# olehskip/resnet.c

Measured on AMD Instinct MI355X. Metric: images/sec ResNet-50 224x224 fp32 batch=256, higher is better.
Workload: dtype f32; 1 GPU; resnet50 fp32 forward, batch 256 per GPU, 224x224 (BASELINE.json configs[2]); global_batch=256, batch_per_gpu=256, mode=fused conv+bn+relu(+add) epilogues, streams_per_gpu=2, streams_configured=library default, front_parts=1, parallelism=batch split over 1 GPU(s), weights replicated, no collective

## Files before the change

resnet.c_amd/csrc/rn_chain.hip:

```cpp
#include "rn_conv_params.h"
#include "rn_lds_dma.h"

using namespace rn_gemm;
using namespace rn_dma;

namespace {

struct ChainParams {
    const void *t2;
    const void *x;
    void *y;
    const void *w3;
    const float *sc3, *sh3;
    void *t1;
    const void *w1;
    const float *sc1, *sh1;
    int M, nsteps;
    int t2_bytes, x_bytes, y_bytes, t1_bytes;
};

typedef bf16_t bf16x4 __attribute__((ext_vector_type(4)));

template <int MID>
struct Geo {
    static constexpr int C = 4 * MID;
    static constexpr int WAVES = MID == 64 ? 8 : 4;
    static constexpr int ROWS = MID == 64 ? 64 : 32;
    static constexpr int PF = ROWS / 32;
    static constexpr int CF1 = C / (32 * WAVES);
    static constexpr int KT2 = MID / 64;
    static constexpr int T2B = ROWS * MID * 2;
    static constexpr int XB = ROWS * C * 2;
    static constexpr int oT2 = 0, oX = 2 * T2B, oY = oX + 2 * XB, oS = oY + XB;
    static constexpr int LDS = oS + (2 * C + 512) * 4;
};

template <int MID, int N1, bool DUAL>
__global__ __launch_bounds__(64 * Geo<MID>::WAVES) void chain_kernel(const ChainParams p)
{
    using G = Geo<MID>;
    constexpr int C = G::C, ROWS = G::ROWS, PF = G::PF, CF1 = G::CF1, THREADS = 64 * G::WAVES;
    constexpr int N1F = N1 / 32;
    static_assert(!DUAL || MID == 64, "pair chain: 64 mid channels");
    static_assert(PF * N1F <= G::WAVES, "one fragment of the second product per wave");
    __shared__ __attribute__((aligned(16))) char lds[G::LDS];
    float *const ssl = reinterpret_cast<float *>(lds + G::oS);
    const int t = threadIdx.x, lane = t & 63;
    const int wave = __builtin_amdgcn_readfirstlane(t >> 6);
    const int li = lane & 31, lh = lane >> 5;

    int nst, s0;
    dealt_range((unsigned)p.nsteps, gridDim.x, blockIdx.x, &nst, &s0);

    const int pf2 = wave % PF, cf2 = wave / PF;
    const bool has2 = cf2 < N1F;
    constexpr int K3S = (DUAL ? 2 : 1) * MID / 16;
    constexpr int K1S = C / 16;
    i32x4 w3r[CF1][K3S], w1r[K1S];
#pragma unroll
    for (int f = 0; f < CF1; ++f) {
        const char *r3 = static_cast<const char *>(p.w3) + (size_t)(32 * (CF1 * wave + f) + li) * (K3S * 32) + lh * 16;
#pragma unroll
        for (int ks = 0; ks < K3S; ++ks) w3r[f][ks] = *reinterpret_cast<const i32x4 *>(r3 + ks * 32);
    }
    {
        const char *r1 = static_cast<const char *>(p.w1) + (size_t)(32 * (has2 ? cf2 : 0) + li) * (K1S * 32) + lh * 16;
#pragma unroll
        for (int s = 0; s < K1S; ++s) w1r[s] = *reinterpret_cast<const i32x4 *>(r1 + s * 32);
    }
    for (int i = t; i < C; i += THREADS) {
        ssl[i] = p.sc3 ? p.sc3[i] : 1.f;
        ssl[C + i] = p.sh3 ? p.sh3[i] : -0.f;
    }
    for (int i = t; i < N1; i += THREADS) {
        ssl[2 * C + i] = p.sc1 ? p.sc1[i] : 1.f;
        ssl[2 * C + 256 + i] = p.sh1 ? p.sh1[i] : -0.f;
    }

    const i32x4 srd_t2 = make_srd(p.t2, p.t2_bytes);
    const i32x4 srd_x = make_srd(p.x, p.x_bytes);
    const __amdgpu_buffer_rsrc_t rsrc_y = make_rsrc(p.y, p.y_bytes);
    const __amdgpu_buffer_rsrc_t rsrc_t1 = make_rsrc(p.t1, p.t1_bytes);
    const unsigned lds_base = (unsigned)(uintptr_t)((lds_void *)lds);

    auto fetch = [&](int s, int buf) {
        const int m0 = (s0 + s) * ROWS;
        const bool live = s < nst;
        constexpr int T2P = G::KT2 * ROWS / 8;
#pragma unroll
        for (int j = 0; j < T2P / G::WAVES; ++j) {
            const int q = G::WAVES * j + wave, kt = q / (ROWS / 8), r = 8 * (q % (ROWS / 8)) + (lane >> 3);
            const int pc = lane & 7, m = m0 + r;
            dma16((live && m < p.M) ? m * (MID * 2) + kt * 128 + (RN_SWZ(pc, r) << 4) : kOob, srd_t2, 0,
                  lds_base + (unsigned)(G::oT2 + buf * G::T2B + q * 1024));
        }
        if constexpr (DUAL) {
#pragma unroll
            for (int j = 0; j < T2P / G::WAVES; ++j) {
                const int q = G::WAVES * j + wave, r = 8 * q + (lane >> 3), pc = lane & 7, m = m0 + r;
                dma16((live && m < p.M) ? m * 128 + (RN_SWZ(pc, r) << 4) : kOob, srd_x, 0,
                      lds_base + (unsigned)(G::oX + buf * G::XB + q * 1024));
            }
        } else {
            constexpr int XP = G::XB / 1024, SPR = C / 8;
#pragma unroll
            for (int j = 0; j < XP / G::WAVES; ++j) {
                const int q = G::WAVES * j + wave, g = 64 * q + lane;
                const int r = g / SPR, sl = g % SPR, m = m0 + r;
                const int c = (sl & ~15) | ((sl & 15) ^ (r & 15));
                dma16((live && m < p.M) ? m * (C * 2) + (c << 4) : kOob, srd_x, 0,
                      lds_base + (unsigned)(G::oX + buf * G::XB + q * 1024));
            }
        }
    };

    fetch(0, 0);
    for (int s = 0; s < nst; ++s) {
        const int buf = s & 1;
        const int m0 = (s0 + s) * ROWS;
        wait_and_barrier<0>();
        if constexpr (MID == 64) fetch(s + 1, buf ^ 1);

        f32x16 acc[PF][CF1];
#pragma unroll
        for (int pf = 0; pf < PF; ++pf)
#pragma unroll
            for (int f = 0; f < CF1; ++f)
#pragma unroll
                for (int e = 0; e < 16; ++e) acc[pf][f][e] = 0.f;
#pragma unroll
        for (int ks = 0; ks < K3S; ++ks) {
#pragma unroll
            for (int pf = 0; pf < PF; ++pf) {
                const int r = 32 * pf + li;
                const bool second = DUAL && ks >= MID / 16;
                const int kk = second ? ks - MID / 16 : ks;
                const char *src = second ? lds + G::oX + buf * G::XB : lds + G::oT2 + buf * G::T2B;
                const i32x4 px = *reinterpret_cast<const i32x4 *>(
                    src + (kk >> 2) * (ROWS * 128) + r * 128 + (RN_SWZ(2 * (kk & 3) + lh, r) << 4));
#pragma unroll
                for (int f = 0; f < CF1; ++f)
                    acc[pf][f] = __builtin_amdgcn_mfma_f32_32x32x16_bf16(__builtin_bit_cast(bf16x8, w3r[f][ks]),
                                                                         __builtin_bit_cast(bf16x8, px), acc[pf][f], 0, 0, 0);
            }
        }
        if constexpr (MID != 64) fetch(s + 1, buf ^ 1);
#pragma unroll
        for (int pf = 0; pf < PF; ++pf)
#pragma unroll
            for (int f = 0; f < CF1; ++f) {
                const int r = 32 * pf + li, cf = CF1 * wave + f;
                unsigned d[4][2];
#pragma unroll
                for (int j = 0; j < 4; ++j) {
                    const int c4 = 32 * cf + 8 * j + 4 * lh;
                    const float4 sc = *reinterpret_cast<const float4 *>(ssl + c4);
                    const float4 sh = *reinterpret_cast<const float4 *>(ssl + C + c4);
                    float4 v = affine4(acc[pf][f], j, sc, sh);
                    if constexpr (!DUAL) {
                        const int chunk = 4 * cf + j;
                        const bf16x4 rv = *reinterpret_cast<const bf16x4 *>(
                            lds + G::oX + buf * G::XB + r * (C * 2) +
                            (((chunk & ~15) | ((chunk & 15) ^ (r & 15))) << 4) + 8 * lh);
                        v.x = v.x + (float)rv[0], v.y = v.y + (float)rv[1], v.z = v.z + (float)rv[2], v.w = v.w + (float)rv[3];
                    }
                    pack_bf16x4(relu4(v), d[j]);
                }
#pragma unroll
                for (int h = 0; h < 2; ++h) {
                    const auto x0 = __builtin_amdgcn_permlane32_swap(d[2 * h][0], d[2 * h + 1][0], false, false);
                    const auto x1 = __builtin_amdgcn_permlane32_swap(d[2 * h][1], d[2 * h + 1][1], false, false);
                    const int cy = 4 * cf + 2 * h + lh;
                    *reinterpret_cast<i32x4 *>(lds + G::oY + (cy >> 3) * (ROWS * 128) + r * 128 +
                                               (RN_SWZ(cy & 7, r) << 4)) =
                        i32x4{(int)x0[0], (int)x1[0], (int)x0[1], (int)x1[1]};
                }
            }
        __syncthreads();

#pragma unroll
        for (int i = 0; i < ROWS * (C / 8) / THREADS; ++i) {
            const int g = t + i * THREADS, r = g / (C / 8), c = g % (C / 8), m = m0 + r;
            const i32x4 v = *reinterpret_cast<const i32x4 *>(lds + G::oY + (c >> 3) * (ROWS * 128) + r * 128 +
                                                             (RN_SWZ(c & 7, r) << 4));
            __builtin_amdgcn_raw_buffer_store_b128(__builtin_bit_cast(u32x4, v), rsrc_y,
                                                   m < p.M ? m * (C * 2) + (c << 4) : kOob, 0, 0);
        }

        if (has2) {
            const int r = 32 * pf2 + li;
            f32x16 a2;
#pragma unroll
            for (int e = 0; e < 16; ++e) a2[e] = 0.f;
#pragma unroll
            for (int s2 = 0; s2 < K1S; ++s2) {
                const i32x4 px = *reinterpret_cast<const i32x4 *>(
                    lds + G::oY + (s2 >> 2) * (ROWS * 128) + r * 128 + (RN_SWZ(2 * (s2 & 3) + lh, r) << 4));
                a2 = __builtin_amdgcn_mfma_f32_32x32x16_bf16(__builtin_bit_cast(bf16x8, w1r[s2]),
                                                             __builtin_bit_cast(bf16x8, px), a2, 0, 0, 0);
            }
            unsigned d[4][2];
#pragma unroll
            for (int j = 0; j < 4; ++j) {
                const int c4 = 32 * cf2 + 8 * j + 4 * lh;
                const float4 sc = *reinterpret_cast<const float4 *>(ssl + 2 * C + c4);
                const float4 sh = *reinterpret_cast<const float4 *>(ssl + 2 * C + 256 + c4);
                pack_bf16x4(affine4_relu(a2, j, sc, sh), d[j]);
            }
            const int m = m0 + r;
#pragma unroll
            for (int h = 0; h < 2; ++h) {
                const auto x0 = __builtin_amdgcn_permlane32_swap(d[2 * h][0], d[2 * h + 1][0], false, false);
                const auto x1 = __builtin_amdgcn_permlane32_swap(d[2 * h][1], d[2 * h + 1][1], false, false);
                const u32x4 o = {x0[0], x1[0], x0[1], x1[1]};
                __builtin_amdgcn_raw_buffer_store_b128(
                    o, rsrc_t1, m < p.M ? (m * N1 + 32 * cf2 + 16 * h + 8 * lh) * 2 : kOob, 0, 0);
            }
        }
    }
}

template <int MID, int N1, bool DUAL>
void chain_go(rn_ctx *ctx, const ChainParams &p)
{
    const int blocks = p.nsteps < 256 ? p.nsteps : 256;
    chain_kernel<MID, N1, DUAL><<<dim3(blocks), dim3(64 * Geo<MID>::WAVES), 0, ctx->stream>>>(p);
}

constexpr int k32XY = 0, k32XYB = 64 * 1024, k32T2 = 2 * k32XYB, k32T2B = 64 * 256;
constexpr int k32S = k32T2 + k32T2B, k32Lds = k32S + (512 + 256) * 4;

template <int N1>
__global__ __launch_bounds__(512) void chain32_kernel(const ChainParams p)
{
    constexpr int ROWS = 64, N1F = N1 / 32;
    __shared__ __attribute__((aligned(16))) char lds[k32Lds];
    float *const ssl = reinterpret_cast<float *>(lds + k32S);
    const int t = threadIdx.x, lane = t & 63;
    const int wave = __builtin_amdgcn_readfirstlane(t >> 6);
    const int li = lane & 31, lh = lane >> 5;
    int nst, s0;
    dealt_range((unsigned)p.nsteps, gridDim.x, blockIdx.x, &nst, &s0);
    const int pf2 = wave & 1, cf2 = wave >> 1;
    const bool has2 = cf2 < N1F;
    u32x4 w3r[2][4], w1r[8][4];
    {
        const char *r3 = static_cast<const char *>(p.w3) + (size_t)(32 * wave + li) * 256 + lh * 16;
#pragma unroll
        for (int kt = 0; kt < 2; ++kt)
#pragma unroll
            for (int ks = 0; ks < 4; ++ks) w3r[kt][ks] = *reinterpret_cast<const u32x4 *>(r3 + kt * 128 + ks * 32);
        const char *r1 = static_cast<const char *>(p.w1) + (size_t)(32 * (has2 ? cf2 : 0) + li) * 1024 + lh * 16;
#pragma unroll
        for (int kt = 0; kt < 8; ++kt)
#pragma unroll
            for (int ks = 0; ks < 4; ++ks) w1r[kt][ks] = *reinterpret_cast<const u32x4 *>(r1 + kt * 128 + ks * 32);
    }
    for (int i = t; i < 256; i += 512) {
        ssl[i] = p.sc3 ? p.sc3[i] : 1.f;
        ssl[256 + i] = p.sh3 ? p.sh3[i] : -0.f;
    }
    for (int i = t; i < N1; i += 512) {
        ssl[512 + i] = p.sc1 ? p.sc1[i] : 1.f;
        ssl[640 + i] = p.sh1 ? p.sh1[i] : -0.f;
    }
    const i32x4 srd_t2 = make_srd(p.t2, p.t2_bytes);
    const i32x4 srd_x = make_srd(p.x, p.x_bytes);
    const __amdgpu_buffer_rsrc_t rsrc_y = make_rsrc(p.y, p.y_bytes);
    const __amdgpu_buffer_rsrc_t rsrc_t1 = make_rsrc(p.t1, p.t1_bytes);
    const unsigned lds_base = (unsigned)(uintptr_t)((lds_void *)lds);
    const int prow = lane >> 3, pc = lane & 7;

    auto fetch_t2 = [&](int s) {
        const int m0 = (s0 + s) * ROWS;
#pragma unroll
        for (int j = 0; j < 2; ++j) {
            const int q = 8 * j + wave, r = 8 * (q & 7) + prow, m = m0 + r;
            dma16((s < nst && m < p.M) ? m * 256 + (q >> 3) * 128 + (RN_SWZ(pc, r) << 4) : kOob, srd_t2, 0,
                  lds_base + (unsigned)(k32T2 + q * 1024));
        }
    };
    auto fetch_x = [&](int s, int buf) {
        const int m0 = (s0 + s) * ROWS;
#pragma unroll
        for (int j = 0; j < 8; ++j) {
            const int q = 8 * j + wave, r = 8 * (q & 7) + prow, m = m0 + r;
            dma16((s < nst && m < p.M) ? m * 1024 + (q >> 3) * 128 + (RN_SWZ(pc, r) << 4) : kOob, srd_x, 0,
                  lds_base + (unsigned)(k32XY + buf * k32XYB + q * 1024));
        }
    };

    fetch_t2(0);
    fetch_x(0, 0);
    for (int s = 0; s < nst; ++s) {
        const int buf = s & 1;
        const int m0 = (s0 + s) * ROWS;
        char *const xy = lds + k32XY + buf * k32XYB;
        wait_and_barrier<0>();
        fetch_x(s + 1, buf ^ 1);

        f32x16 acc[2];
#pragma unroll
        for (int pf = 0; pf < 2; ++pf)
#pragma unroll
            for (int e = 0; e < 16; ++e) acc[pf][e] = 0.f;
#pragma unroll
        for (int pf = 0; pf < 2; ++pf)
#pragma unroll
            for (int kt = 0; kt < 2; ++kt)
#pragma unroll
                for (int ks = 0; ks < 4; ++ks) {
                    const int r = 32 * pf + li;
                    const u32x4 px = *reinterpret_cast<const u32x4 *>(
                        lds + k32T2 + kt * 8192 + r * 128 + (RN_SWZ(2 * ks + lh, r) << 4));
#pragma unroll
                    for (int j = 0; j < 4; ++j)
                        acc[pf] = __builtin_amdgcn_mfma_f32_32x32x2f32(__uint_as_float(w3r[kt][ks][j]),
                                                                        __uint_as_float(px[j]), acc[pf], 0, 0, 0);
                }
#pragma unroll
        for (int pf = 0; pf < 2; ++pf) {
            const int r = 32 * pf + li;
#pragma unroll
            for (int g = 0; g < 4; ++g) {
                const int c4 = 32 * wave + 8 * g + 4 * lh;
                const float4 sc = *reinterpret_cast<const float4 *>(ssl + c4);
                const float4 sh = *reinterpret_cast<const float4 *>(ssl + 256 + c4);
                float4 *slot = reinterpret_cast<float4 *>(xy + wave * 8192 + r * 128 + (RN_SWZ(2 * g + lh, r) << 4));
                const float4 rv = *slot;
                *slot = affine4_add_relu(acc[pf], g, sc, sh, rv);
            }
        }
        __syncthreads();
        fetch_t2(s + 1);

        {
            constexpr bool kSplit = N1F == 2;
            const int tt = kSplit ? t - 256 : t;
            if (!kSplit || wave >= 4) {
#pragma unroll 1
                for (int i0 = 0; i0 < (kSplit ? 16 : 8); i0 += 4) {
#pragma unroll
                    for (int i = i0; i < i0 + 4; ++i) {
                        const int g = tt + i * (kSplit ? 256 : 512), r = g >> 6, c = g & 63, m = m0 + r;
                        const u32x4 v = *reinterpret_cast<const u32x4 *>(xy + (c >> 3) * 8192 + r * 128 +
                                                                         (RN_SWZ(c & 7, r) << 4));
                        __builtin_amdgcn_raw_buffer_store_b128(v, rsrc_y, m < p.M ? m * 1024 + (c << 4) : kOob, 0, 0);
                    }
                }
            }
        }

        if (has2) {
            const int r = 32 * pf2 + li;
            f32x16 a2;
#pragma unroll
            for (int e = 0; e < 16; ++e) a2[e] = 0.f;
#pragma unroll
            for (int kt = 0; kt < 8; ++kt)
#pragma unroll
                for (int ks = 0; ks < 4; ++ks) {
                    const u32x4 px = *reinterpret_cast<const u32x4 *>(
                        xy + kt * 8192 + r * 128 + (RN_SWZ(2 * ks + lh, r) << 4));
#pragma unroll
                    for (int j = 0; j < 4; ++j)
                        a2 = __builtin_amdgcn_mfma_f32_32x32x2f32(__uint_as_float(w1r[kt][ks][j]), __uint_as_float(px[j]),
                                                                  a2, 0, 0, 0);
                }
            const int m = m0 + r;
#pragma unroll
            for (int g = 0; g < 4; ++g) {
                const int c4 = 32 * cf2 + 8 * g + 4 * lh;
                const float4 sc = *reinterpret_cast<const float4 *>(ssl + 512 + c4);
                const float4 sh = *reinterpret_cast<const float4 *>(ssl + 640 + c4);
                const u32x4 o = __builtin_bit_cast(u32x4, affine4_relu(a2, g, sc, sh));
                __builtin_amdgcn_raw_buffer_store_b128(o, rsrc_t1, m < p.M ? (m * N1 + c4) * 4 : kOob, 0, 0);
            }
        }
    }
}

constexpr int kP32Y = 0, kP32W1 = 64 * 1024, kP32T2 = 128 * 1024, kP32X2 = 144 * 1024, kP32Lds = 160 * 1024;

__global__ __launch_bounds__(512) void chain32_pair_kernel(const ChainParams p)
{
    constexpr int ROWS = 64;
    __shared__ __attribute__((aligned(16))) char lds[kP32Lds];
    const int t = threadIdx.x, lane = t & 63;
    const int wave = __builtin_amdgcn_readfirstlane(t >> 6);
    const int li = lane & 31, lh = lane >> 5;
    int nst, s0;
    dealt_range((unsigned)p.nsteps, gridDim.x, blockIdx.x, &nst, &s0);
    const int pf2 = wave & 1, cf2 = wave >> 1;
    const bool has2 = cf2 < 2;
    u32x4 w3r[4][4];
    {
        const char *r3 = static_cast<const char *>(p.w3) + (size_t)(32 * wave + li) * 512 + lh * 16;
#pragma unroll
        for (int kt = 0; kt < 4; ++kt)
#pragma unroll
            for (int ks = 0; ks < 4; ++ks) w3r[kt][ks] = *reinterpret_cast<const u32x4 *>(r3 + kt * 128 + ks * 32);
    }
    const i32x4 srd_t2 = make_srd(p.t2, p.t2_bytes);
    const i32x4 srd_x = make_srd(p.x, p.x_bytes);
    const i32x4 srd_w1 = make_srd(p.w1, 64 * 256 * 4);
    const __amdgpu_buffer_rsrc_t rsrc_y = make_rsrc(p.y, p.y_bytes);
    const __amdgpu_buffer_rsrc_t rsrc_t1 = make_rsrc(p.t1, p.t1_bytes);
    const unsigned lds_base = (unsigned)(uintptr_t)((lds_void *)lds);
    const int prow = lane >> 3, pc = lane & 7;

#pragma unroll
    for (int j = 0; j < 8; ++j) {
        const int q = 8 * j + wave, r = 8 * (q & 7) + prow;
        dma16(r * 1024 + (q >> 3) * 128 + (RN_SWZ(pc, r) << 4), srd_w1, 0,
              lds_base + (unsigned)(kP32W1 + q * 1024));
    }
    auto fetch_in = [&](int s) {
        const int m0 = (s0 + s) * ROWS;
#pragma unroll
        for (int j = 0; j < 2; ++j) {
            const int q = 8 * j + wave, r = 8 * (q & 7) + prow, m = m0 + r;
            const int off = (s < nst && m < p.M) ? m * 256 + (q >> 3) * 128 + (RN_SWZ(pc, r) << 4) : kOob;
            dma16(off, srd_t2, 0, lds_base + (unsigned)(kP32T2 + q * 1024));
            dma16(off, srd_x, 0, lds_base + (unsigned)(kP32X2 + q * 1024));
        }
    };

    fetch_in(0);
    for (int s = 0; s < nst; ++s) {
        const int m0 = (s0 + s) * ROWS;
        wait_and_barrier<0>();

        f32x16 acc[2];
#pragma unroll
        for (int pf = 0; pf < 2; ++pf)
#pragma unroll
            for (int e = 0; e < 16; ++e) acc[pf][e] = 0.f;
#pragma unroll
        for (int pf = 0; pf < 2; ++pf)
#pragma unroll
            for (int kt = 0; kt < 4; ++kt)
#pragma unroll
                for (int ks = 0; ks < 4; ++ks) {
                    const int r = 32 * pf + li;
                    const u32x4 px = *reinterpret_cast<const u32x4 *>(
                        lds + (kt < 2 ? kP32T2 : kP32X2) + (kt & 1) * 8192 + r * 128 + (RN_SWZ(2 * ks + lh, r) << 4));
#pragma unroll
                    for (int j = 0; j < 4; ++j)
                        acc[pf] = __builtin_amdgcn_mfma_f32_32x32x2f32(__uint_as_float(w3r[kt][ks][j]),
                                                                        __uint_as_float(px[j]), acc[pf], 0, 0, 0);
                }
#pragma unroll
        for (int pf = 0; pf < 2; ++pf) {
            const int r = 32 * pf + li;
#pragma unroll
            for (int g = 0; g < 4; ++g) {
                const int c4 = 32 * wave + 8 * g + 4 * lh;
                const float4 sh = p.sh3 ? *reinterpret_cast<const float4 *>(p.sh3 + c4) : make_float4(-0.f, -0.f, -0.f, -0.f);
                const float4 o = affine4_relu(acc[pf], g, make_float4(1.f, 1.f, 1.f, 1.f), sh);
                *reinterpret_cast<float4 *>(lds + kP32Y + wave * 8192 + r * 128 + (RN_SWZ(2 * g + lh, r) << 4)) = o;
            }
        }
        __syncthreads();
        fetch_in(s + 1);

        if (wave >= 4) {
#pragma unroll 1
            for (int i0 = 0; i0 < 16; i0 += 4) {
#pragma unroll
                for (int i = i0; i < i0 + 4; ++i) {
                    const int g = t - 256 + i * 256, r = g >> 6, c = g & 63, m = m0 + r;
                    const u32x4 v = *reinterpret_cast<const u32x4 *>(lds + kP32Y + (c >> 3) * 8192 + r * 128 +
                                                                     (RN_SWZ(c & 7, r) << 4));
                    __builtin_amdgcn_raw_buffer_store_b128(v, rsrc_y, m < p.M ? m * 1024 + (c << 4) : kOob, 0, 0);
                }
            }
        }

        if (has2) {
            const int r = 32 * pf2 + li, wr = 32 * cf2 + li;
            f32x16 a2;
#pragma unroll
            for (int e = 0; e < 16; ++e) a2[e] = 0.f;
#pragma unroll
            for (int kt = 0; kt < 8; ++kt)
#pragma unroll
                for (int ks = 0; ks < 4; ++ks) {
                    const u32x4 px = *reinterpret_cast<const u32x4 *>(
                        lds + kP32Y + kt * 8192 + r * 128 + (RN_SWZ(2 * ks + lh, r) << 4));
                    const u32x4 wv = *reinterpret_cast<const u32x4 *>(
                        lds + kP32W1 + kt * 8192 + wr * 128 + (RN_SWZ(2 * ks + lh, wr) << 4));
#pragma unroll
                    for (int j = 0; j < 4; ++j)
                        a2 = __builtin_amdgcn_mfma_f32_32x32x2f32(__uint_as_float(wv[j]), __uint_as_float(px[j]), a2, 0, 0, 0);
                }
            const int m = m0 + r;
#pragma unroll
            for (int g = 0; g < 4; ++g) {
                const int c4 = 32 * cf2 + 8 * g + 4 * lh;
                const float4 sc = p.sc1 ? *reinterpret_cast<const float4 *>(p.sc1 + c4) : make_float4(1.f, 1.f, 1.f, 1.f);
                const float4 sh = p.sh1 ? *reinterpret_cast<const float4 *>(p.sh1 + c4) : make_float4(-0.f, -0.f, -0.f, -0.f);
                const u32x4 o = __builtin_bit_cast(u32x4, affine4_relu(a2, g, sc, sh));
                __builtin_amdgcn_raw_buffer_store_b128(o, rsrc_t1, m < p.M ? (m * 64 + c4) * 4 : kOob, 0, 0);
            }
        }
    }
}

int chain_launch(rn_ctx *ctx, const char *what, int dtype, const void *t2, const void *x, bool dual, void *y,
                 const void *w3, const float *scale3, const float *shift3, void *t1, const void *w1,
                 const float *scale1, const float *shift1, uint64_t rows, uint64_t mid_channels,
                 uint64_t channels, uint64_t next_mid)
{
    if (rows == 0) return RN_OK;
    RN_REQUIRE(ctx, dtype == RN_DTYPE_BF16 || dtype == RN_DTYPE_F32, "unknown dtype");
    RN_REQUIRE(ctx, t2 && x && y && w3 && t1 && w1, "null tensor");
    RN_REQUIRE(ctx, ((reinterpret_cast<uintptr_t>(t2) | reinterpret_cast<uintptr_t>(x) | reinterpret_cast<uintptr_t>(y) |
                      reinterpret_cast<uintptr_t>(t1) | reinterpret_cast<uintptr_t>(w3) | reinterpret_cast<uintptr_t>(w1) |
                      reinterpret_cast<uintptr_t>(scale3) | reinterpret_cast<uintptr_t>(shift3) |
                      reinterpret_cast<uintptr_t>(scale1) | reinterpret_cast<uintptr_t>(shift1)) & 15) == 0,
               "tensors, panels and scale / shift vectors must be 16-byte aligned");
    RN_REQUIRE(ctx, y != t1 && y != t2 && y != x && t1 != t2 && t1 != x, "y and t1 must not alias each other or an input");
    const bool s1 = mid_channels == 64 && channels == 256 && (next_mid == 64 || next_mid == 128);
    const bool s2 = mid_channels == 128 && channels == 512 && next_mid == 128 && !dual && dtype == RN_DTYPE_BF16;
    RN_REQUIRE(ctx, s1 || s2, "shapes: 64 -> 256 -> 64 | 128 channels, or (bf16) 128 -> 512 -> 128");
    RN_REQUIRE(ctx, !(dual && dtype == RN_DTYPE_F32 && next_mid != 64), "fp32 pair chain: next_mid 64");
    const uint64_t es = rn_elem_size(dtype);
    RN_REQUIRE(ctx, rows * channels * es < (1ull << 31), "tensor too large");
    if (dtype == RN_DTYPE_F32) {
        ChainParams q;
        q.t2 = t2, q.x = x, q.y = y, q.w3 = w3, q.sc3 = scale3, q.sh3 = shift3;
        q.t1 = t1, q.w1 = w1, q.sc1 = scale1, q.sh1 = shift1;
        q.M = (int)rows;
        q.nsteps = (int)((rows + 63) / 64);
        q.t2_bytes = (int)(rows * 256), q.x_bytes = q.y_bytes = (int)(rows * 1024), q.t1_bytes = (int)(rows * next_mid * 4);
        const dim3 grid(q.nsteps < 256 ? q.nsteps : 256), block(512);
        if (dual) {
            q.x_bytes = (int)(rows * 256);
            chain32_pair_kernel<<<grid, block, 0, ctx->stream>>>(q);
        } else if (next_mid == 64)
            chain32_kernel<64><<<grid, block, 0, ctx->stream>>>(q);
        else
            chain32_kernel<128><<<grid, block, 0, ctx->stream>>>(q);
        return rn_after_launch(ctx, what);
    }
    ChainParams p;
    p.t2 = t2, p.x = x, p.y = y, p.w3 = w3, p.sc3 = scale3, p.sh3 = shift3;
    p.t1 = t1, p.w1 = w1, p.sc1 = scale1, p.sh1 = shift1;
    p.M = (int)rows;
    const uint64_t step = s1 ? 64 : 32;
    p.nsteps = (int)((rows + step - 1) / step);
    p.t2_bytes = (int)(rows * mid_channels * 2), p.x_bytes = (int)(rows * (dual ? 128 : channels * 2));
    p.y_bytes = (int)(rows * channels * 2), p.t1_bytes = (int)(rows * next_mid * 2);
    if (s2)
        chain_go<128, 128, false>(ctx, p);
    else if (dual)
        next_mid == 64 ? chain_go<64, 64, true>(ctx, p) : chain_go<64, 128, true>(ctx, p);
    else
        next_mid == 64 ? chain_go<64, 64, false>(ctx, p) : chain_go<64, 128, false>(ctx, p);
    return rn_after_launch(ctx, what);
}

}

extern "C" {

int rn_conv_chain_forward_dt(rn_ctx *ctx, int dtype, const void *t2, const void *residual, void *y,
                             const void *packed_w3, const float *scale3, const float *shift3,
                             void *t1, const void *packed_w1, const float *scale1, const float *shift1,
                             uint64_t rows, uint64_t mid_channels, uint64_t channels, uint64_t next_mid)
{
    RN_ENTER(ctx);
    return chain_launch(ctx, "rn_conv_chain_forward_dt", dtype, t2, residual, false, y, packed_w3, scale3, shift3,
                        t1, packed_w1, scale1, shift1, rows, mid_channels, channels, next_mid);
}

int rn_conv_chain_pair_forward_dt(rn_ctx *ctx, int dtype, const void *t2, const void *x2, void *y,
                                  const void *packed_pair, const float *shift, void *t1,
                                  const void *packed_w1, const float *scale1, const float *shift1,
                                  uint64_t rows, uint64_t mid_channels, uint64_t in2_channels,
                                  uint64_t channels, uint64_t next_mid)
{
    RN_ENTER(ctx);
    RN_REQUIRE(ctx, in2_channels == 64, "second input: 64 channels");
    return chain_launch(ctx, "rn_conv_chain_pair_forward_dt", dtype, t2, x2, true, y, packed_pair, nullptr, shift,
                        t1, packed_w1, scale1, shift1, rows, mid_channels, channels, next_mid);
}

}
```

Measured before the change: 15230 images/s.

## Overlap conv3 epilogue, y export and DMA waits with MFMA in fp32 chain kernels

Reworks the fp32 chain kernels' per-step schedule. Full vmcnt(0) barriers become partial DMA waits, and the next x prefetch now issues after the first MFMA group. The conv3 BN/residual epilogue for the first row half runs interleaved with the second half's MFMAs, and the y export is split across conv1 MFMA iterations with double-buffered LDS loads. It also reorders the DMA row mapping, hoists scale/shift vectors into registers in the pair kernel, and adds an optional timestamp instrumentation path. The aim is to hide LDS, epilogue and store latency behind matrix ops, at the cost of register pressure and fragile hand-counted waitcnt values.

```diff
diff --git a/resnet.c_amd/csrc/rn_chain.hip b/resnet.c_amd/csrc/rn_chain.hip
--- a/resnet.c_amd/csrc/rn_chain.hip
+++ b/resnet.c_amd/csrc/rn_chain.hip
@@ -230,8 +230,104 @@
 constexpr int k32XY = 0, k32XYB = 64 * 1024, k32T2 = 2 * k32XYB, k32T2B = 64 * 256;
 constexpr int k32S = k32T2 + k32T2B, k32Lds = k32S + (512 + 256) * 4;
 
-template <int N1>
-__global__ __launch_bounds__(512) void chain32_kernel(const ChainParams p)
+template <int AFTER>
+__device__ __forceinline__ void wait_dma(bool first)
+{
+    if (first)
+        asm volatile("s_waitcnt vmcnt(0)" ::: "memory");
+    else
+        asm volatile("s_waitcnt vmcnt(%0)" ::"n"(AFTER) : "memory");
+}
+__device__ __forceinline__ void lds_barrier()
+{
+    asm volatile("s_waitcnt lgkmcnt(0)\n\ts_barrier" ::: "memory");
+    __builtin_amdgcn_sched_barrier(0);
+}
+
+__device__ __forceinline__ void settle(float4 &v)
+{
+    asm volatile("" : "+v"(v.x), "+v"(v.y), "+v"(v.z), "+v"(v.w));
+}
+
+template <int NW>
+struct ExportY {
+    const char *lds0;
+    __amdgpu_buffer_rsrc_t rsrc_y;
+    int tile_off, m0, M, first;
+    int lrow, lane_lds, lane_glb;
+    bool whole;
+    __device__ __forceinline__ ExportY(const char *lds0_, int tile_off_, __amdgpu_buffer_rsrc_t rsrc, int m0_, int M_, int first_,
+                                       int lane)
+        : lds0(lds0_), rsrc_y(rsrc), tile_off(tile_off_), m0(m0_), M(M_), first(first_), lrow((lane >> 3) & 1),
+          lane_lds((lane >> 4) * 8192 + lrow * 128 + ((lane & 7) << 4)),
+          lane_glb(lrow * 1024 + (lane >> 4) * 128 + ((lane & 7) << 4)), whole(m0_ + 64 <= M_)
+    {
+    }
+    __device__ __forceinline__ void read(int i0, u32x4 (&v)[4]) const
+    {
+#pragma unroll
+        for (int i = 0; i < 4; ++i) {
+            const int u = first + (i0 + i) * NW, rp = u >> 1;
+            v[i] = *reinterpret_cast<const u32x4 *>(
+                lds0 + (lane_lds ^ (tile_off + (u & 1) * 32768 + rp * 256 + ((rp & 7) << 4))));
+        }
+    }
+    __device__ __forceinline__ void store(int i0, const u32x4 (&v)[4]) const
+    {
+        if (whole) {
+#pragma unroll
+            for (int i = 0; i < 4; ++i) {
+                const int u = first + (i0 + i) * NW, m = m0 + 2 * (u >> 1);
+                __builtin_amdgcn_raw_buffer_store_b128(v[i], rsrc_y, lane_glb, m * 1024 + (u & 1) * 512, 0);
+            }
+        } else {
+#pragma unroll
+            for (int i = 0; i < 4; ++i) {
+                const int u = first + (i0 + i) * NW, m = m0 + 2 * (u >> 1);
+                __builtin_amdgcn_raw_buffer_store_b128(v[i], rsrc_y, m + lrow < M ? m * 1024 + (u & 1) * 512 + lane_glb : kOob, 0, 0);
+            }
+        }
+    }
+    __device__ __forceinline__ void all() const
+    {
+#pragma unroll 1
+        for (int i0 = 0; i0 < 64 / NW; i0 += 4) {
+            u32x4 v[4];
+            read(i0, v);
+            store(i0, v);
+        }
+    }
+};
+
+constexpr int kStampStep = 2, kStampSlots = 9;
+struct Chain32Params : ChainParams {
+    unsigned long long *stamps;
+};
+template <bool STAMP>
+struct Stamps {
+    unsigned long long tk[kStampSlots] = {};
+    __device__ __forceinline__ void at(int s, int slot)
+    {
+        if constexpr (STAMP) {
+            if (s == kStampStep) {
+                __builtin_amdgcn_sched_barrier(0);
+                tk[slot] = __builtin_amdgcn_s_memtime();
+                __builtin_amdgcn_sched_barrier(0);
+            }
+        }
+    }
+    __device__ __forceinline__ void write(unsigned long long *out, int wave, int lane) const
+    {
+        if constexpr (STAMP) {
+            if (out && lane == 0 && tk[kStampSlots - 1])
+#pragma unroll
+                for (int i = 0; i < kStampSlots; ++i) out[((size_t)blockIdx.x * 8 + wave) * 16 + i] = tk[i];
+        }
+    }
+};
+
+template <int N1, bool STAMP>
+__global__ __launch_bounds__(512) void chain32_kernel(const Chain32Params p)
 {
     constexpr int ROWS = 64, N1F = N1 / 32;
     __shared__ __attribute__((aligned(16))) char lds[k32Lds];
@@ -275,8 +371,8 @@
         const int m0 = (s0 + s) * ROWS;
 #pragma unroll
         for (int j = 0; j < 2; ++j) {
-            const int q = 8 * j + wave, r = 8 * (q & 7) + prow, m = m0 + r;
-            dma16((s < nst && m < p.M) ? m * 256 + (q >> 3) * 128 + (RN_SWZ(pc, r) << 4) : kOob, srd_t2, 0,
+            const int q = 8 * j + wave, r = 8 * wave + prow, m = m0 + r;
+            dma16((s < nst && m < p.M) ? m * 256 + (RN_SWZ(pc, r) << 4) : kOob, srd_t2, j * 128,
                   lds_base + (unsigned)(k32T2 + q * 1024));
         }
     };
@@ -284,105 +380,143 @@
         const int m0 = (s0 + s) * ROWS;
 #pragma unroll
         for (int j = 0; j < 8; ++j) {
-            const int q = 8 * j + wave, r = 8 * (q & 7) + prow, m = m0 + r;
-            dma16((s < nst && m < p.M) ? m * 1024 + (q >> 3) * 128 + (RN_SWZ(pc, r) << 4) : kOob, srd_x, 0,
+            const int q = 8 * j + wave, r = 8 * wave + prow, m = m0 + r;
+            dma16((s < nst && m < p.M) ? m * 1024 + (RN_SWZ(pc, r) << 4) : kOob, srd_x, j * 128,
                   lds_base + (unsigned)(k32XY + buf * k32XYB + q * 1024));
         }
     };
 
+    constexpr bool kSplit = N1F == 2;
+    Stamps<STAMP> st;
     fetch_t2(0);
     fetch_x(0, 0);
     for (int s = 0; s < nst; ++s) {
         const int buf = s & 1;
         const int m0 = (s0 + s) * ROWS;
         char *const xy = lds + k32XY + buf * k32XYB;
-        wait_and_barrier<0>();
-        fetch_x(s + 1, buf ^ 1);
+        if (kSplit && wave >= 4)
+            wait_dma<16>(s == 0);
+        else
+            wait_dma<kSplit ? 4 : 12>(s == 0);
+        lds_barrier();
+        st.at(s - 1, 8);
+        st.at(s, 0);
 
         f32x16 acc[2];
 #pragma unroll
         for (int pf = 0; pf < 2; ++pf)
 #pragma unroll
             for (int e = 0; e < 16; ++e) acc[pf][e] = 0.f;
+        st.at(s, 1);
+        auto slot_of = [&](int pf, int g) {
+            const int r = 32 * pf + li;
+            return reinterpret_cast<float4 *>(xy + wave * 8192 + r * 128) + RN_SWZ(2 * g + lh, r);
+        };
+        auto cst = [&](int g, float4 &sc, float4 &sh) {
+            const int c4 = 32 * wave + 8 * g + 4 * lh;
+            sc = *reinterpret_cast<const float4 *>(ssl + c4), sh = *reinterpret_cast<const float4 *>(ssl + 256 + c4);
+        };
+        float4 rv1, sc, sh, rv[4];
 #pragma unroll
         for (int pf = 0; pf < 2; ++pf)
 #pragma unroll
-            for (int kt = 0; kt < 2; ++kt)
-#pragma unroll
-                for (int ks = 0; ks < 4; ++ks) {
-                    const int r = 32 * pf + li;
-                    const u32x4 px = *reinterpret_cast<const u32x4 *>(
-                        lds + k32T2 + kt * 8192 + r * 128 + (RN_SWZ(2 * ks + lh, r) << 4));
-#pragma unroll
-                    for (int j = 0; j < 4; ++j)
-                        acc[pf] = __builtin_amdgcn_mfma_f32_32x32x2f32(__uint_as_float(w3r[kt][ks][j]),
-                                                                        __uint_as_float(px[j]), acc[pf], 0, 0, 0);
-                }
-#pragma unroll
-        for (int pf = 0; pf < 2; ++pf) {
-            const int r = 32 * pf + li;
-#pragma unroll
-            for (int g = 0; g < 4; ++g) {
-                const int c4 = 32 * wave + 8 * g + 4 * lh;
-                const float4 sc = *reinterpret_cast<const float4 *>(ssl + c4);
-                const float4 sh = *reinterpret_cast<const float4 *>(ssl + 256 + c4);
-                float4 *slot = reinterpret_cast<float4 *>(xy + wave * 8192 + r * 128 + (RN_SWZ(2 * g + lh, r) << 4));
-                const float4 rv = *slot;
-                *slot = affine4_add_relu(acc[pf], g, sc, sh, rv);
-            }
-        }
+            for (int gi = 0; gi < 8; ++gi) {
+                const int kt = gi >> 2, ks = gi & 3;
+                const int r = 32 * pf + li;
+                const u32x4 px = *reinterpret_cast<const u32x4 *>(
+                    lds + k32T2 + kt * 8192 + r * 128 + (RN_SWZ(2 * ks + lh, r) << 4));
+                if (pf == 1 && gi <= 4) {
+                    if (gi >= 1) *slot_of(0, gi - 1) = affine4_add_relu(acc[0], gi - 1, sc, sh, rv1);
+                    if (gi <= 3) rv1 = *slot_of(0, gi), cst(gi, sc, sh);
+                    __builtin_amdgcn_sched_barrier(0);
+                }
+                if (pf == 1 && gi == 6) {
+#pragma unroll
+                    for (int g = 0; g < 4; ++g) rv[g] = *slot_of(1, g);
+                    cst(0, sc, sh);
+                    __builtin_amdgcn_sched_barrier(0);
+                }
+#pragma unroll
+                for (int j = 0; j < 4; ++j)
+                    acc[pf] = __builtin_amdgcn_mfma_f32_32x32x2f32(__uint_as_float(w3r[kt][ks][j]),
+                                                                    __uint_as_float(px[j]), acc[pf], 0, 0, 0);
+                if (pf == 1 && (gi <= 4 || gi == 6)) __builtin_amdgcn_sched_barrier(0);
+                if (pf == 0 && gi == 0) {
+                    __builtin_amdgcn_sched_barrier(0);
+                    fetch_x(s + 1, buf ^ 1);
+                    __builtin_amdgcn_sched_barrier(0);
+                }
+            }
+        st.at(s, 2);
+#pragma unroll
+        for (int g = 0; g < 4; ++g) {
+            if (g) cst(g, sc, sh);
+            rv[g] = affine4_add_relu(acc[1], g, sc, sh, rv[g]);
+        }
+#pragma unroll
+        for (int g = 0; g < 4; ++g) *slot_of(1, g) = rv[g];
+        st.at(s, 3);
         __syncthreads();
+        st.at(s, 4);
         fetch_t2(s + 1);
 
-        {
-            constexpr bool kSplit = N1F == 2;
-            const int tt = kSplit ? t - 256 : t;
-            if (!kSplit || wave >= 4) {
-#pragma unroll 1
-                for (int i0 = 0; i0 < (kSplit ? 16 : 8); i0 += 4) {
-#pragma unroll
-                    for (int i = i0; i < i0 + 4; ++i) {
-                        const int g = tt + i * (kSplit ? 256 : 512), r = g >> 6, c = g & 63, m = m0 + r;
-                        const u32x4 v = *reinterpret_cast<const u32x4 *>(xy + (c >> 3) * 8192 + r * 128 +
-                                                                         (RN_SWZ(c & 7, r) << 4));
-                        __builtin_amdgcn_raw_buffer_store_b128(v, rsrc_y, m < p.M ? m * 1024 + (c << 4) : kOob, 0, 0);
-                    }
-                }
-            }
-        }
+        static_assert(kSplit || N1F == 4, "unsplit: every wave has a fragment of conv1 to export beside");
+        if constexpr (kSplit) {
+            if (wave >= 4) ExportY<4>(lds, k32XY + buf * k32XYB, rsrc_y, m0, p.M, wave - 4, lane).all();
+        }
+        const ExportY<8> ex(lds, k32XY + buf * k32XYB, rsrc_y, m0, p.M, wave, lane);
+        u32x4 ev[4];
+        st.at(s, 5);
 
         if (has2) {
             const int r = 32 * pf2 + li;
             f32x16 a2;
 #pragma unroll
             for (int e = 0; e < 16; ++e) a2[e] = 0.f;
-#pragma unroll
-            for (int kt = 0; kt < 8; ++kt)
-#pragma unroll
-                for (int ks = 0; ks < 4; ++ks) {
-                    const u32x4 px = *reinterpret_cast<const u32x4 *>(
-                        xy + kt * 8192 + r * 128 + (RN_SWZ(2 * ks + lh, r) << 4));
-#pragma unroll
-                    for (int j = 0; j < 4; ++j)
-                        a2 = __builtin_amdgcn_mfma_f32_32x32x2f32(__uint_as_float(w1r[kt][ks][j]), __uint_as_float(px[j]),
-                                                                  a2, 0, 0, 0);
-                }
+            const char *const yrow = xy + r * 128;
+            u32x4 px[2];
+            float4 sc1v[4], sh1v[4];
+            px[0] = *reinterpret_cast<const u32x4 *>(yrow + (RN_SWZ(lh, r) << 4));
+#pragma unroll
+            for (int q = 0; q < 32; ++q) {
+                if constexpr (!kSplit) {
+                    if (q == 0 || q == 4) ex.read(q, ev);
+                    if (q == 2 || q == 6) ex.store(q - 2, ev);
+                }
+                if (q == 30) {
+#pragma unroll
+                    for (int g = 0; g < 4; ++g) {
+                        const int c4 = 32 * cf2 + 8 * g + 4 * lh;
+                        sc1v[g] = *reinterpret_cast<const float4 *>(ssl + 512 + c4);
+                        sh1v[g] = *reinterpret_cast<const float4 *>(ssl + 640 + c4);
+                    }
+                }
+                if (q + 1 < 32)
+                    px[(q + 1) & 1] = *reinterpret_cast<const u32x4 *>(
+                        yrow + ((q + 1) >> 2) * 8192 + (RN_SWZ(2 * ((q + 1) & 3) + lh, r) << 4));
+#pragma unroll
+                for (int j = 0; j < 4; ++j)
+                    a2 = __builtin_amdgcn_mfma_f32_32x32x2f32(__uint_as_float(w1r[q >> 2][q & 3][j]),
+                                                              __uint_as_float(px[q & 1][j]), a2, 0, 0, 0);
+            }
+            st.at(s, 6);
             const int m = m0 + r;
 #pragma unroll
             for (int g = 0; g < 4; ++g) {
                 const int c4 = 32 * cf2 + 8 * g + 4 * lh;
-                const float4 sc = *reinterpret_cast<const float4 *>(ssl + 512 + c4);
-                const float4 sh = *reinterpret_cast<const float4 *>(ssl + 640 + c4);
-                const u32x4 o = __builtin_bit_cast(u32x4, affine4_relu(a2, g, sc, sh));
+                const u32x4 o = __builtin_bit_cast(u32x4, affine4_relu(a2, g, sc1v[g], sh1v[g]));
                 __builtin_amdgcn_raw_buffer_store_b128(o, rsrc_t1, m < p.M ? (m * N1 + c4) * 4 : kOob, 0, 0);
             }
         }
-    }
+        st.at(s, 7);
+    }
+    st.write(p.stamps, wave, lane);
 }
 
 constexpr int kP32Y = 0, kP32W1 = 64 * 1024, kP32T2 = 128 * 1024, kP32X2 = 144 * 1024, kP32Lds = 160 * 1024;
 
-__global__ __launch_bounds__(512) void chain32_pair_kernel(const ChainParams p)
+template <bool STAMP>
+__global__ __launch_bounds__(512) void chain32_pair_kernel(const Chain32Params p)
 {
     constexpr int ROWS = 64;
     __shared__ __attribute__((aligned(16))) char lds[kP32Lds];
@@ -426,16 +560,40 @@
         }
     };
 
+    float4 sh3r[4], sc1r[4], sh1r[4];
+#pragma unroll
+    for (int g = 0; g < 4; ++g) {
+        const int c3 = 32 * wave + 8 * g + 4 * lh, c1 = 32 * (has2 ? cf2 : 0) + 8 * g + 4 * lh;
+        sh3r[g] = p.sh3 ? *reinterpret_cast<const float4 *>(p.sh3 + c3) : make_float4(-0.f, -0.f, -0.f, -0.f);
+        sc1r[g] = p.sc1 ? *reinterpret_cast<const float4 *>(p.sc1 + c1) : make_float4(1.f, 1.f, 1.f, 1.f);
+        sh1r[g] = p.sh1 ? *reinterpret_cast<const float4 *>(p.sh1 + c1) : make_float4(-0.f, -0.f, -0.f, -0.f);
+    }
+#pragma unroll
+    for (int g = 0; g < 4; ++g) settle(sh3r[g]), settle(sc1r[g]), settle(sh1r[g]);
+
+    Stamps<STAMP> st;
     fetch_in(0);
     for (int s = 0; s < nst; ++s) {
         const int m0 = (s0 + s) * ROWS;
-        wait_and_barrier<0>();
+        if (wave >= 4)
+            wait_dma<16>(s == 0);
+        else
+            wait_dma<4>(s == 0);
+        lds_barrier();
+        st.at(s - 1, 8);
+        st.at(s, 0);
+        st.at(s, 1);
 
         f32x16 acc[2];
 #pragma unroll
         for (int pf = 0; pf < 2; ++pf)
 #pragma unroll
             for (int e = 0; e < 16; ++e) acc[pf][e] = 0.f;
+        auto finish = [&](int pf, int g) {
+            const int r = 32 * pf + li;
+            const float4 o = affine4_relu(acc[pf], g, make_float4(1.f, 1.f, 1.f, 1.f), sh3r[g]);
+            *reinterpret_cast<float4 *>(lds + kP32Y + wave * 8192 + r * 128 + (RN_SWZ(2 * g + lh, r) << 4)) = o;
+        };
 #pragma unroll
         for (int pf = 0; pf < 2; ++pf)
 #pragma unroll
@@ -445,37 +603,26 @@
                     const int r = 32 * pf + li;
                     const u32x4 px = *reinterpret_cast<const u32x4 *>(
                         lds + (kt < 2 ? kP32T2 : kP32X2) + (kt & 1) * 8192 + r * 128 + (RN_SWZ(2 * ks + lh, r) << 4));
+                    if (pf == 1 && kt == 0) {
+                        __builtin_amdgcn_sched_barrier(0);
+                        finish(0, ks);
+                        __builtin_amdgcn_sched_barrier(0);
+                    }
 #pragma unroll
                     for (int j = 0; j < 4; ++j)
                         acc[pf] = __builtin_amdgcn_mfma_f32_32x32x2f32(__uint_as_float(w3r[kt][ks][j]),
                                                                         __uint_as_float(px[j]), acc[pf], 0, 0, 0);
                 }
-#pragma unroll
-        for (int pf = 0; pf < 2; ++pf) {
-            const int r = 32 * pf + li;
-#pragma unroll
-            for (int g = 0; g < 4; ++g) {
-                const int c4 = 32 * wave + 8 * g + 4 * lh;
-                const float4 sh = p.sh3 ? *reinterpret_cast<const float4 *>(p.sh3 + c4) : make_float4(-0.f, -0.f, -0.f, -0.f);
-                const float4 o = affine4_relu(acc[pf], g, make_float4(1.f, 1.f, 1.f, 1.f), sh);
-                *reinterpret_cast<float4 *>(lds + kP32Y + wave * 8192 + r * 128 + (RN_SWZ(2 * g + lh, r) << 4)) = o;
-            }
-        }
+        st.at(s, 2);
+#pragma unroll
+        for (int g = 0; g < 4; ++g) finish(1, g);
+        st.at(s, 3);
         __syncthreads();
+        st.at(s, 4);
         fetch_in(s + 1);
 
-        if (wave >= 4) {
-#pragma unroll 1
-            for (int i0 = 0; i0 < 16; i0 += 4) {
-#pragma unroll
-                for (int i = i0; i < i0 + 4; ++i) {
-                    const int g = t - 256 + i * 256, r = g >> 6, c = g & 63, m = m0 + r;
-                    const u32x4 v = *reinterpret_cast<const u32x4 *>(lds + kP32Y + (c >> 3) * 8192 + r * 128 +
-                                                                     (RN_SWZ(c & 7, r) << 4));
-                    __builtin_amdgcn_raw_buffer_store_b128(v, rsrc_y, m < p.M ? m * 1024 + (c << 4) : kOob, 0, 0);
-                }
-            }
-        }
+        if (wave >= 4) ExportY<4>(lds, kP32Y, rsrc_y, m0, p.M, wave - 4, lane).all();
+        st.at(s, 5);
 
         if (has2) {
             const int r = 32 * pf2 + li, wr = 32 * cf2 + li;
@@ -494,17 +641,18 @@
                     for (int j = 0; j < 4; ++j)
                         a2 = __builtin_amdgcn_mfma_f32_32x32x2f32(__uint_as_float(wv[j]), __uint_as_float(px[j]), a2, 0, 0, 0);
                 }
+            st.at(s, 6);
             const int m = m0 + r;
 #pragma unroll
             for (int g = 0; g < 4; ++g) {
                 const int c4 = 32 * cf2 + 8 * g + 4 * lh;
-                const float4 sc = p.sc1 ? *reinterpret_cast<const float4 *>(p.sc1 + c4) : make_float4(1.f, 1.f, 1.f, 1.f);
-                const float4 sh = p.sh1 ? *reinterpret_cast<const float4 *>(p.sh1 + c4) : make_float4(-0.f, -0.f, -0.f, -0.f);
-                const u32x4 o = __builtin_bit_cast(u32x4, affine4_relu(a2, g, sc, sh));
+                const u32x4 o = __builtin_bit_cast(u32x4, affine4_relu(a2, g, sc1r[g], sh1r[g]));
                 __builtin_amdgcn_raw_buffer_store_b128(o, rsrc_t1, m < p.M ? (m * 64 + c4) * 4 : kOob, 0, 0);
             }
         }
-    }
+        st.at(s, 7);
+    }
+    st.write(p.stamps, wave, lane);
 }
 
 int chain_launch(rn_ctx *ctx, const char *what, int dtype, const void *t2, const void *x, bool dual, void *y,
@@ -528,20 +676,19 @@
     const uint64_t es = rn_elem_size(dtype);
     RN_REQUIRE(ctx, rows * channels * es < (1ull << 31), "tensor too large");
     if (dtype == RN_DTYPE_F32) {
-        ChainParams q;
+        Chain32Params q;
         q.t2 = t2, q.x = x, q.y = y, q.w3 = w3, q.sc3 = scale3, q.sh3 = shift3;
         q.t1 = t1, q.w1 = w1, q.sc1 = scale1, q.sh1 = shift1;
         q.M = (int)rows;
         q.nsteps = (int)((rows + 63) / 64);
         q.t2_bytes = (int)(rows * 256), q.x_bytes = q.y_bytes = (int)(rows * 1024), q.t1_bytes = (int)(rows * next_mid * 4);
+        q.stamps = (unsigned long long *)ctx->debug_stamps;
         const dim3 grid(q.nsteps < 256 ? q.nsteps : 256), block(512);
-        if (dual) {
-            q.x_bytes = (int)(rows * 256);
-            chain32_pair_kernel<<<grid, block, 0, ctx->stream>>>(q);
-        } else if (next_mid == 64)
-            chain32_kernel<64><<<grid, block, 0, ctx->stream>>>(q);
-        else
-            chain32_kernel<128><<<grid, block, 0, ctx->stream>>>(q);
+        if (dual) q.x_bytes = (int)(rows * 256);
+        auto *const kernel = dual            ? (q.stamps ? chain32_pair_kernel<true> : chain32_pair_kernel<false>)
+                             : next_mid == 64 ? (q.stamps ? chain32_kernel<64, true> : chain32_kernel<64, false>)
+                                              : (q.stamps ? chain32_kernel<128, true> : chain32_kernel<128, false>);
+        kernel<<<grid, block, 0, ctx->stream>>>(q);
         return rn_after_launch(ctx, what);
     }
     ChainParams p;
```

New measurement: 15330 images/s (median of 4 runs). About the same (+0.7%).
